# ehsan5890/optical-rl-gym-qot-aware

Hardware: AMD Instinct MI355X
Metric: env steps/sec (whole node) + blocking-prob parity, NSFNET RMSA 320 slots (higher is better)
Workload: dtype u64 bitmap + f64 statistics

## Files before the change

### optical-rl-gym-qot-aware_amd/csrc/orlg_api_step.hip

```cpp
#include "orlg_rmsa_host.h"
#include "orlg_step_call.h"
#include "orlg_qdesc.h"

typedef orlg_rmsa_kernel_t rmsa_kernel_t;

static OrlgGroupOverrides group_overrides() {
    const char *wpb = getenv("ORLG_GROUP_WPB"), *chunks = getenv("ORLG_GROUP_CHUNKS");
    return {getenv("ORLG_NO_DEFER") != nullptr, getenv("ORLG_NO_CHUNKS") != nullptr, getenv("ORLG_NO_LEAN") != nullptr,
            wpb ? atoi(wpb) : 0, chunks ? atoi(chunks) : 0};
}

static bool usage_launch(const OrlgParams &p) {
    return (p.out_mask & ORLG_OUT_ASSIGN_BIT) != 0 && (p.assign == ORLG_ASSIGN_MOST_USED || p.policy == ORLG_POLICY_BEST_WINDOW);
}

static int launch_rmsa_group(orlg_env *e, const OrlgParams &p, const OrlgGroupOverrides &ov) {
    OrlgGroupChoice c = orlg_group_choose(e->group, {p.B, p.n_steps, p.stats_level, p.policy, p.out_mask, p.br_width}, ov, e->num_cu);
    const OrlgGroupLayout &l = e->group[c.kind];
    const bool df = c.kind == ORLG_GROUP_DEFER;
    const bool trace = p.tr_arrival != nullptr;
    const bool traffic = !trace && p.rates != nullptr;
    const bool cause = (p.out_mask & ORLG_OUT_CAUSE_BIT) != 0;
    const bool assign = (p.out_mask & ORLG_OUT_ASSIGN_BIT) != 0;
    const bool cut = assign && p.assign == ORLG_ASSIGN_MIN_CUT;
    const bool usage = usage_launch(p);
    const OrlgGroupKey key = {p.stats_level, c.kind == ORLG_GROUP_HBMQ, df, traffic, trace, cause, assign, cut, usage};
    rmsa_kernel_t k = orlg_pick(e->W, key);
    if (!k) return fail(ORLG_ERR_INVALID, "no kernel for W=%d", e->W);
    if (usage) {
        c.wpb = orlg_group_usage_wpb(l, c.wpb, e->W);
        if (c.wpb < 1)
            return fail(ORLG_ERR_INVALID, "step_kernel \"group\": one wave's four environments (%d B) and their slot-usage prefix sums (%d B) do not "
                                          "fit the LDS next to the tables (%d B); use step_kernel \"wave\" or \"auto\" for this policy",
                        l.wave_bytes, 4 * ORLG_USAGE_BYTES(e->W), l.shared_bytes);
        c.lds_bytes = orlg_group_lds(l.shared_bytes, c.wpb, l.wave_bytes + 4 * ORLG_USAGE_BYTES(e->W));
    }
    if (df && !e->llog)
        if (int rc = orlg_handle_alloc(e, &e->llog, (size_t)p.B * p.E * ORLG_LLOG_CAP)) return rc;
    if (int rc = orlg_kernel_lds(reinterpret_cast<const void *>(k), usage ? c.lds_bytes : orlg_group_lds(l.shared_bytes, l.wpb_max, l.wave_bytes))) return rc;
    int *resident = usage ? &e->group_usage_resident[c.wpb] : &e->group_resident[c.kind][c.wpb];
    if (int rc = orlg_handle_resident(e, reinterpret_cast<const void *>(k), ORLG_WAVE * c.wpb, c.lds_bytes, resident)) return rc;
    const OrlgGroupTickets t = orlg_group_tickets(c, p.B, p.n_steps, *resident, ov);
    if (t.n_chunks > 1) {
        if (!e->progress)
            if (int rc = orlg_handle_alloc(e, &e->progress, (size_t)p.B / 4 + 1)) return rc;
        HIP_TRY(hipMemsetAsync(e->progress, 0, (size_t)t.n_quads * sizeof(uint32_t), e->stream));
    }
    OrlgParams q = p;
    q.llog = df ? e->llog : nullptr;
    q.g_lstat = l.lstat; q.g_lint = l.lint; q.g_qtime = l.qtime; q.g_qdesc = l.qdesc; q.g_wave_bytes = l.wave_bytes;
// ... 403 lines not shown
```

### optical-rl-gym-qot-aware_amd/csrc/orlg_group_body.h

```cpp
    static_assert(!DEFER || (STATS >= 2 && !HBMQ), "the deferred link statistics belong to long launches with full statistics");
    static_assert(!(TRACE && TRAFFIC), "a trace handle has no arrival rates");
    static_assert(!LEAN || DEFER, "the lean body belongs to the long launches");
    static_assert(!CAUSE || (!HBMQ && !DEFER), "the blocking cause belongs to the plain kind");
    static_assert(!ASSIGN || (!HBMQ && !DEFER), "the assignment rules belong to the plain kind");
    static_assert(!CUT || ASSIGN, "the fewest-cuts window is an assignment rule");
    static_assert(!USAGE || (ASSIGN && !CUT), "most-used windows and the best-window route are assignment rules of their own");
    extern __shared__ __align__(16) unsigned char smem[];
    stage_tables(smem, p);
    const int lane = threadIdx.x & 63;
    const int wib = uni((int)(threadIdx.x >> 6));
    const int g = lane >> 4, gl = lane & 15;
    const Tab tb = make_tab(smem, p);
    uint32_t *mt_lds = reinterpret_cast<uint32_t *>(smem + p.l_shared_bytes);
    int *mt_lock = reinterpret_cast<int *>(smem + p.l_shared_bytes + p.g_mt);
    if (threadIdx.x == 0) *mt_lock = 0;
    __syncthreads();
    unsigned char *wbase = smem + p.l_shared_bytes + p.g_mt + 16 + (size_t)wib * p.g_wave_bytes;
    u64 *occ = reinterpret_cast<u64 *>(wbase + p.g_occ) + g * p.NW;
    double *qtime = nullptr;
    uint32_t *qdesc = nullptr;
    if constexpr (!HBMQ) {
        qtime = reinterpret_cast<double *>(wbase + p.g_qtime) + g * p.Q;
        qdesc = reinterpret_cast<uint32_t *>(wbase + p.g_qdesc) + g * p.Q;
    }
    double *lst = DEFER ? nullptr : reinterpret_cast<double *>(wbase + p.g_lstat) + g * 4 * p.E;
    int32_t *lint = reinterpret_cast<int32_t *>(wbase + p.g_lint) + g * p.lint_stride;
    u64 *lsum = DEFER ? reinterpret_cast<u64 *>(wbase + p.g_lstat) + g * p.E : nullptr;

    const int E = p.E, S = p.S, K = p.K, N = p.N, NBR = p.NBR, Q = p.Q, NW = p.NW;
    constexpr bool NET = STATS >= 1;
    constexpr bool FULL = STATS >= 2;
    const double INF = __longlong_as_double((long long)ORLG_INF_BITS);
    const bool out_comp = !LEAN && (p.out_mask & ((1 << ORLG_OUT_COMPACT) | (1 << ORLG_OUT_COMPACT_DIFF))) != 0;
    SEC_DECL_G

    const int n_quads = (p.B + ORLG_GE - 1) / ORLG_GE;
    const int n_chunks = p.n_chunks > 1 ? p.n_chunks : 1;
    const int n_tix = n_quads * n_chunks;
    const int n_waves = (int)(gridDim.x * (blockDim.x >> 6));
// ... 24 lines not shown
        __builtin_amdgcn_fence(__ATOMIC_ACQUIRE, "agent");
        asm volatile("s_waitcnt vmcnt(0)" ::: "memory");
    }
    const int env_raw = quad * ORLG_GE + g;
    const bool act = env_raw < p.B;
    const int env = act ? env_raw : p.B - 1;

    const int env0 = quad * ORLG_GE;
    const int nact = p.B - env0 < ORLG_GE ? p.B - env0 : ORLG_GE;
    quad_copy(wbase + p.g_occ, p.occ + (size_t)env0 * NW, nact * NW * 8, lane);
    if (FULL && !DEFER) quad_copy(wbase + p.g_lstat, p.lstat + (size_t)env0 * 4 * E, nact * 4 * E * 8, lane);
    int32_t *ghist = p.hist + (size_t)env * 4 * NBR;
    [[maybe_unused]] char *hist_q = reinterpret_cast<char *>(p.hist + (size_t)env0 * 4 * NBR);
    [[maybe_unused]] const uint32_t hist_row = (uint32_t)((env - env0) * 4 * NBR) * 4u;
    [[maybe_unused]] auto hist_at = [&](int which, int i) -> int32_t * {
        return reinterpret_cast<int32_t *>(hist_q + (hist_row + (uint32_t)(which * NBR + i) * 4u));
    };
    if (NET) quad_copy(wbase + p.g_lint, p.lint + (size_t)env0 * p.lint_stride, nact * p.lint_stride * 4, lane);
    if (nact < ORLG_GE) {
        wave_sync();
        if (!act) {
            const int gs_ = nact - 1;
            for (int i = gl; i < NW; i += ORLG_GL) occ[i] = (reinterpret_cast<u64 *>(wbase + p.g_occ) + gs_ * NW)[i];
            if (FULL && !DEFER) for (int i = gl; i < 4 * E; i += ORLG_GL) lst[i] = (reinterpret_cast<double *>(wbase + p.g_lstat) + gs_ * 4 * E)[i];
            if (NET) for (int i = gl; i < p.lint_stride; i += ORLG_GL) lint[i] = (reinterpret_cast<int32_t *>(wbase + p.g_lint) + gs_ * p.lint_stride)[i];
        }
    }
    uint4 *llog = DEFER ? p.llog + (size_t)env * E * ORLG_LLOG_CAP : nullptr;
    if (DEFER) lst = p.lstat + (size_t)env * 4 * E;
    bool need_replay = false;
    const OrlgEnvScalars *gs = p.scal + env;
    double current_time = gs->current_time, req_arrival = gs->req_arrival, req_holding = gs->req_holding;
    double g_thr = gs->g_throughput, g_comp = gs->g_compactness, g_lu = gs->g_last_update;
    long long cnt = gs->c[gl & 7];
    long long sum_bitrate_running = gs->sum_bitrate_running, episodes_done = gs->episodes_done;
    int sum_sh = gs->sum_slots_hops, n_running = gs->n_running;
    int req_src = gs->req_src, req_dst = gs->req_dst, req_br = gs->req_br, req_sid = gs->req_sid;
    int mt_idx = gs->mt_idx, new_service = gs->new_service, q_overflow = gs->q_overflow;
    int ring_pos = gs->ring_pos, ring_cnt = gs->ring_cnt;
    int sum_span = gs->sum_span, sum_gaps = gs->sum_gaps;
    int eproc = (int)gs->c[2];
    wave_sync();
    [[maybe_unused]] OrlgGraphEntry lg = {0.0, 0u, 0u, 0u};
    [[maybe_unused]] int lg_cnt = 0;
    double comp_cur = 1.0;
    if (NET && !LEAN) comp_cur = network_compactness(sum_span, sum_sh, sum_gaps, E);
    if (DEFER)
        group_link_stats<W, true, false, true, 2>(lane, occ, nullptr, lint, tb, S, E, nullptr, E, 0.0, sum_span, sum_gaps, comp_cur,
                                                  0, 0.0, g_thr, g_comp, g_lu, nullptr, nullptr, lsum);
    int q_head = gs->q_head, q_n = n_running < Q ? n_running : Q;
    const int q_head0 = q_head;
    int q_pops = 0;
    if constexpr (HBMQ) {
        qtime = p.qtime + (size_t)env * Q;
        qdesc = p.qdesc + (size_t)env * Q;
    } else {
        const double *gqt = p.qtime + (size_t)env * Q;
        const uint32_t *gqd = p.qdesc + (size_t)env * Q;
        for (int j = gl; j < q_n; j += 2 * ORLG_GL) {
            int pos = q_head + j;
            pos -= pos >= Q ? Q : 0;
            int pos2 = pos + ORLG_GL;
            pos2 -= pos2 >= Q ? Q : 0;
            const bool two = j + ORLG_GL < q_n;
            const double t0 = gqt[pos];
            const uint32_t d0 = gqd[pos];
            double t1 = 0.0;
            uint32_t d1 = 0u;
            if (two) { t1 = gqt[pos2]; d1 = gqd[pos2]; }
            qtime[pos] = t0; qdesc[pos] = d0;
            if (two) { qtime[pos2] = t1; qdesc[pos2] = d1; }
        }
    }
    wave_sync();
    double next_rel = q_n > 0 ? qtime[q_head] : INF;
// ... 188 lines not shown
        const double prev_compact = comp_cur;
        bool accepted = false;
        const bool in_range = act && a_path >= 0 && a_path < K && a_slot >= 0 && a_slot < S;
        const int gid = base + (in_range ? a_path : 0);
        const OrlgPathRec *rec = tb.recs + gid;
        int hops = ff_hops, n = ff_n;
        if (LEAN || policy != ORLG_POLICY_EXT) {
            accepted = in_range;
        } else {
            hops = rec->hops;
            n = tb.nslots[req_br * ORLG_NSLOT_STRIDE + rec->se];
            const bool on = in_range && gl < W;
            const u64 x = path_word<W>(occ, tb.recs, gid, gl < W ? gl : 0, on);
            const u64 m = on ? window_mask(a_slot, n, gl) : 0ull;
            const uint32_t bad = row_ballot((x & m) != m, lane);
            accepted = in_range && a_slot + n <= S && bad == 0u;
        }
        const int br_val = tb.bit_rates[req_br];
        [[maybe_unused]] int cause = 0;
        if constexpr (CAUSE) {
            const bool refused = act && !accepted;
            if (ballot(refused) != 0ull) {
                const int level = group_fit_level<W>(lane, occ, tb, base, K, S, req_br, refused);
                cause = refused ? ORLG_CAUSE_CAPACITY + level : ORLG_CAUSE_ACCEPTED;
            }
            if (act) cause_cnt += gl == cause ? 1 : 0;
        }
        if (!NET) group_apply_window<W>(lane, occ, rec->link, accepted ? hops : 0, a_slot, n, false);
        if constexpr (DEFER) vm_drain();
        if (accepted) {
            sum_sh += n * hops;
            n_running += 1;
            sum_bitrate_running += br_val;
            cnt += (cidx == 1 || cidx == 3) ? 1 : ((cidx == 5 || cidx == 7) ? br_val : 0);
            if constexpr (DEFER) {
                if (gl == 0) { atomicAdd(hist_at(1, req_br), 1); atomicAdd(hist_at(3, req_br), 1); }
            } else {
                if (gl == 0) { atomicAdd(ghist + NBR + req_br, 1); atomicAdd(ghist + 3 * NBR + req_br, 1); }
            }
        }
        SEC(4);
        if (NET)
            group_link_stats<W, FULL, !LEAN, DEFER, DEFER ? 1 : 0, true>(lane, occ, lst, lint, tb, S, E, rec->link, accepted ? hops : 0,
                                                                           current_time, sum_span, sum_gaps, comp_cur, sum_sh,
                                                                           (double)sum_bitrate_running, g_thr, g_comp, g_lu, llog,
                                                                           &need_replay, lsum, a_slot, n);
        if constexpr (LEAN) {
            const bool logs = accepted && hops > 0;
            OrlgGraphEntry ne;
            orlg_glog_pack(ne, current_time, sum_bitrate_running, sum_span, sum_sh, sum_gaps);
            if (logs && gl == lg_cnt) lg = ne;
            lg_cnt += logs ? 1 : 0;
            if (ballot(lg_cnt >= ORLG_GLOG_CAP) != 0ull) {
                SEC(15);
                group_graph_replay(lane, lg, lg_cnt, p.scal + env, E);
                vm_drain();
            }
        }
        SEC(5);
        {
            const double rel = req_arrival + req_holding;
            bool ins = accepted && (act || !HBMQ);
            if (ins && q_n >= Q) { q_overflow = 1; ins = false; }
            bool down = false;
            if constexpr (!HBMQ) {
                if (ins && q_n > 0) {
                    int pm = q_head + (q_n >> 1);
                    pm -= pm >= Q ? Q : 0;
                    down = rel < qtime[pm];
                }
            }
            bool found = !ins || q_n == 0;
            int m = q_n;
            int left = q_n;
            int j = down ? gl : q_n - 1 - gl;
            int hd = down ? q_head - 1 : q_head + 1;
            hd = hd < 0 ? Q - 1 : (hd == Q ? 0 : hd);
            while (ballot(!found) != 0ull) {
                const bool scan = !found;
                const bool valid = scan && gl < left;
                int pos = q_head + j;
                pos -= pos >= Q ? Q : 0;
                double tq = 0.0;
// ... 90 lines not shown
                                                  arrival_lambda, holding_lambda)
                    : refill_requests<false>(mt_lds, p.ring_iat + (size_t)env_s * ORLG_RING, p.ring_ht + (size_t)env_s * ORLG_RING,
                                             p.ring_req + (size_t)env_s * ORLG_RING, tb.src_cum, tb.dst_cum, tb.br_cum, &idx_s, N,
                                             NBR, arrival_lambda, holding_lambda, env_s);
                m0 = l_mt[lane]; m1 = l_mt[lane + 64];
                if (lane < 156 - 128) m2 = l_mt[lane + 128];
                __builtin_amdgcn_fence(__ATOMIC_RELEASE, "workgroup");
                if (lane == 0) atomicExch(mt_lock, 0);
                uint4 *o_mt = reinterpret_cast<uint4 *>(p.mt + (size_t)env_s * ORLG_MT_N);
                o_mt[lane] = m0; o_mt[lane + 64] = m1;
                if (lane < 156 - 128) o_mt[lane + 128] = m2;
                ring_visible();
                if constexpr (DEFER) vm_drain();
                if ((lane & 48) == src_lane) { ring_cnt = got; ring_pos = 0; mt_idx = idx_s; dry = false; }
            }
            SEC(7);
            double r_iat = pf_iat, r_ht = pf_ht;
            uint32_t rq = pf_rq;
            if (!pf_ok) {
                const size_t ro = (size_t)env * ORLG_RING + ring_pos;
                r_iat = p.ring_iat[ro]; r_ht = p.ring_ht[ro]; rq = p.ring_req[ro];
                if constexpr (DEFER) vm_drain();
            }
            if (act) {
                const double at = TRACE ? r_iat : current_time + r_iat;
                ring_pos += 1; ring_cnt -= 1;
                current_time = at;
                req_src = (int)(rq & 0xffu); req_dst = (int)((rq >> 8) & 0xffu); req_br = (int)(rq >> 16);
                req_base = tb.pair_base[req_src * N + req_dst];
                req_sid = eproc;
                new_service = 1;
                eproc += 1;
                req_arrival = at; req_holding = r_ht;
                const int bv = tb.bit_rates[req_br];
                cnt += (cidx == 0 || cidx == 2) ? 1 : ((cidx == 4 || cidx == 6) ? bv : 0);
                if constexpr (DEFER) {
                    if (gl == 0) { atomicAdd(hist_at(0, req_br), 1); atomicAdd(hist_at(2, req_br), 1); }
                } else {
                    if (gl == 0) { atomicAdd(ghist + req_br, 1); atomicAdd(ghist + 2 * NBR + req_br, 1); }
                }
            }

            bool released = false;
            for (;;) {
                SEC(9);
                const bool rel_now = act && next_rel <= current_time;
                if (ballot(rel_now) == 0ull) break;
                SEC(10);
                if constexpr (DEFER) {
                    const uint32_t d_a = rel_now ? next_desc : 0u;
                    const uint4 rec_a = *reinterpret_cast<const uint4 *>(tb.recs + (int)(d_a & 0x3fff));
                    double b_rel = INF;
                    uint32_t b_desc = 0u;
                    if (rel_now && q_n >= 2) {
                        const int qb = q_head + 1 == Q ? 0 : q_head + 1;
                        b_rel = qtime[qb]; b_desc = qdesc[qb];
                    }
                    const bool b_due = b_rel <= current_time;
                    const int bri_a = (int)(d_a >> 24);
                    int r_link, r_hop, r_hops, r_s, r_n, pops, br_out, sh_out;
                    if (ballot(b_due) == 0ull) {
                        r_hops = rel_now ? (int)(rec_a.x & 0xffu) : 0;
                        r_n = tb.nslots[bri_a * ORLG_NSLOT_STRIDE + (int)((rec_a.x >> 8) & 0xffu)];
                        br_out = tb.bit_rates[bri_a];
                        r_link = group_rec_byte(rec_a, (gl + 2) & 15);
                        r_hop = gl;
                        r_s = (int)((d_a >> 14) & 0x3ff);
                        pops = 1;
                        sh_out = r_n * r_hops;
                    } else {
                        const bool up = gl >= 8;
                        const bool mine = up ? b_due : rel_now;
// ... 3 lines not shown
                        const OrlgPathRec *rec2 = tb.recs + (int)(d & 0x3fff);
                        const int hops2 = mine ? (int)rec2->hops : 0;
                        const int n2 = tb.nslots[bri2 * ORLG_NSLOT_STRIDE + rec2->se];
                        const int br2 = mine ? tb.bit_rates[bri2] : 0;
                        const int link2 = (int)rec2->link[hop];
                        const u64 lbits = half_row_or_u64(hop < hops2 ? 1ull << (link2 & 63) : 0ull);
                        const u64 obits = ((u64)(uint32_t)row_swap8_i32((int)(uint32_t)(lbits >> 32)) << 32) | (uint32_t)row_swap8_i32((int)(uint32_t)lbits);
                        const int hops_o = row_swap8_i32(hops2), n_o = row_swap8_i32(n2), br_o = row_swap8_i32(br2);
                        const bool pair = b_due && hops2 <= 8 && hops_o <= 8 && (lbits & obits) == 0ull;
                        const bool a_up = up && !pair;
                        const int hops_a = up ? hops_o : hops2, n_a = up ? n_o : n2, br_a = up ? br_o : br2;
                        const int hops_b = up ? hops2 : hops_o, n_b = up ? n2 : n_o, br_b = up ? br2 : br_o;
                        r_link = a_up ? group_rec_byte(rec_a, (gl + 2) & 15) : link2;
                        r_hop = pair ? hop : gl;
                        r_hops = a_up ? hops_a : hops2;
                        r_s = a_up ? (int)((d_a >> 14) & 0x3ff) : s0;
                        r_n = a_up ? n_a : n2;
                        pops = pair ? 2 : 1;
                        br_out = br_a + (pair ? br_b : 0);
                        sh_out = n_a * hops_a + (pair ? n_b * hops_b : 0);
                    }
                    if (rel_now) {
                        q_head += pops;
                        q_head -= q_head >= Q ? Q : 0;
                        q_pops += pops;
                        q_n -= pops;
                        n_running -= pops;
                        sum_bitrate_running -= br_out;
                        sum_sh -= sh_out;
                        released = true;
                        next_rel = q_n > 0 ? qtime[q_head] : INF;
                        next_desc = q_n > 0 ? qdesc[q_head] : 0u;
                    }
                    group_release_links<W>(lane, occ, lsum, lint, S, r_link, r_hop, r_hops, r_s, r_n, current_time, sum_span, sum_gaps,
                                           llog, need_replay);
                    SEC(11);
                } else {
                    const uint32_t d = rel_now ? next_desc : 0u;
                    const int gid2 = (int)(d & 0x3fff), s0 = (int)((d >> 14) & 0x3ff), bri2 = (int)(d >> 24);
                    const OrlgPathRec *rec2 = tb.recs + gid2;
                    const int hops2 = rec2->hops;
                    const int n2 = tb.nslots[bri2 * ORLG_NSLOT_STRIDE + rec2->se];
                    if (rel_now) {
                        if (HBMQ && gl == 0) { qtime[q_head] = INF; qdesc[q_head] = 0u; }
                        q_head = q_head + 1 == Q ? 0 : q_head + 1;
                        q_pops += 1;
                        q_n -= 1;
                        n_running -= 1;
                        sum_bitrate_running -= tb.bit_rates[bri2];
                        sum_sh -= n2 * hops2;
                        released = true;
                    }
                    group_apply_window<W>(lane, occ, rec2->link, rel_now ? hops2 : 0, s0, n2, true);
                    if (rel_now) {
                        next_rel = q_n > 0 ? qtime[q_head] : INF;
                        next_desc = q_n > 0 ? qdesc[q_head] : 0u;
                    }
                    SEC(11);
                    if (NET)
                        group_link_stats<W, FULL, false, DEFER>(lane, occ, lst, lint, tb, S, E, rec2->link, rel_now ? hops2 : 0,
                                                                current_time, sum_span, sum_gaps, comp_cur, sum_sh, 0.0, g_thr, g_comp,
                                                                g_lu, llog, &need_replay);
                }
                if (DEFER && ballot(need_replay) != 0ull) {
                    SEC(14);
                    group_link_replay(lane, lst, lint, tb, S, E, llog);
                    vm_drain();
                    need_replay = false;
                    SEC(11);
                }
            }
            if (NET && out_comp && released) comp_cur = network_compactness(sum_span, sum_sh, sum_gaps, E);
        }

        if (DEFER && ballot(need_replay) != 0ull) {
            SEC(14);
            group_link_replay(lane, lst, lint, tb, S, E, llog);
            vm_drain();
            need_replay = false;
        }
        SEC(12);
        {
            const bool done = act && eproc == p.episode_length;
            if (!LEAN && act && gl == 0 && (p.out_mask & (1 << ORLG_OUT_DONE)))
                ORLG_GPTR(uint8_t, tb.outs[ORLG_OUT_DONE])[(size_t)(t0 + t) * p.B + env] = done ? 1 : 0;
            if (ballot(done && p.auto_reset)) {
                if (done && p.auto_reset) {
                    if constexpr (DEFER) {
                        for (int i = gl; i < NBR; i += ORLG_GL) { atomicExch(hist_at(2, i), 0); atomicExch(hist_at(3, i), 0); }
                    } else {
                        for (int i = gl; i < NBR; i += ORLG_GL) { atomicExch(ghist + 2 * NBR + i, 0); atomicExch(ghist + 3 * NBR + i, 0); }
                    }
                    eproc = 1;
                    episodes_done += 1;
                    const int bv = tb.bit_rates[req_br];
                    if (cidx == 2) cnt = 1;
                    if (cidx == 3 || cidx == 7) cnt = 0;
                    if (cidx == 6) cnt = bv;
                }
                wave_sync();
                if constexpr (DEFER) {
                    if (done && p.auto_reset && gl == 0) atomicExch(hist_at(2, req_br), 1);
                } else {
                    if (done && p.auto_reset && gl == 0) atomicExch(ghist + 2 * NBR + req_br, 1);
                }
                wave_sync();
            }
        }
    }

    SEC(14);
    if (DEFER) group_link_replay(lane, lst, lint, tb, S, E, llog);
    if constexpr (LEAN) {
        SEC(15);
        if (ballot(lg_cnt > 0) != 0ull) group_graph_replay(lane, lg, lg_cnt, p.scal + env, E);
    }
    SEC(13);
    wave_sync();
    {
        const int env0 = quad * ORLG_GE;
        const int nact = p.B - env0 < ORLG_GE ? p.B - env0 : ORLG_GE;
        quad_copy(p.occ + (size_t)env0 * NW, wbase + p.g_occ, nact * NW * 8, lane);
        if (FULL && !DEFER) quad_copy(p.lstat + (size_t)env0 * 4 * E, wbase + p.g_lstat, nact * 4 * E * 8, lane);
        if (NET) quad_copy(p.lint + (size_t)env0 * p.lint_stride, wbase + p.g_lint, nact * p.lint_stride * 4, lane);
    }
    if constexpr (CAUSE) {
        if (act && gl < ORLG_NUM_CAUSES && cause_cnt && p.o_cause_counts) atomicAdd(p.o_cause_counts + (size_t)env * ORLG_NUM_CAUSES + gl, cause_cnt);
    }
    if (act) {
        int q_headc = q_head;
        if constexpr (!HBMQ) {
            double *gqt = p.qtime + (size_t)env * Q;
            uint32_t *gqd = p.qdesc + (size_t)env * Q;
            q_headc = q_head0 + (int)((uint32_t)q_pops % (uint32_t)Q);
            q_headc -= q_headc >= Q ? Q : 0;
            int span = q_pops + q_n;
            span = span > Q ? Q : span;
            for (int j = gl; j < span; j += ORLG_GL) {
                int pos = q_head0 + j;
                pos -= pos >= Q ? Q : 0;
                int i = pos - q_headc;
                i += i < 0 ? Q : 0;
                int src = q_head + i;
                src -= src >= Q ? Q : 0;
                double tq = INF;
                uint32_t dq = 0u;
                if (i < q_n) { tq = qtime[src]; dq = qdesc[src]; }
                gqt[pos] = tq; gqd[pos] = dq;
            }
        }
        OrlgEnvScalars *go = p.scal + env;
        if (gl < 8) go->c[gl] = cnt;
        if (gl == 8) {
            go->current_time = current_time;
            go->req_arrival = req_arrival; go->req_holding = req_holding;
            if (!LEAN) { go->g_throughput = g_thr; go->g_compactness = g_comp; go->g_last_update = g_lu; }
            go->sum_bitrate_running = sum_bitrate_running;
            go->episodes_done = episodes_done;
            go->sum_slots_hops = sum_sh; go->n_running = n_running;
            go->req_src = req_src; go->req_dst = req_dst; go->req_br = req_br; go->req_sid = req_sid;
            go->mt_idx = mt_idx; go->new_service = new_service; go->q_overflow = q_overflow;
            go->ring_pos = ring_pos; go->ring_cnt = ring_cnt;
            go->sum_span = sum_span; go->sum_gaps = sum_gaps; go->q_head = q_headc;
            if (q_overflow) *p.err_flag = 1;
        }
    }
    wave_sync();
    if (n_chunks > 1) {
        asm volatile("s_waitcnt vmcnt(0)" ::: "memory");
        __builtin_amdgcn_fence(__ATOMIC_RELEASE, "agent");
        asm volatile("s_waitcnt vmcnt(0)" ::: "memory");
        if (lane == 0) __hip_atomic_store(p.progress + quad, (uint32_t)(chunk + 1), __ATOMIC_RELAXED, __HIP_MEMORY_SCOPE_AGENT);
    }
    SEC(0);
    }
    SEC_FLUSH;
```

### optical-rl-gym-qot-aware_amd/csrc/orlg_group_kernels.hip

```cpp
#pragma once
#include "orlg_link_stats.h"
#include "orlg_requests.h"
#include "orlg_sections.h"
#include "orlg_block_cause.h"
#include "orlg_assign.h"
#include "orlg_cut.h"
#include "orlg_usage.h"
#include "orlg_graph_log.h"

#define ORLG_GL 16
#define ORLG_GE 4

DEV int row_add_i32(int v) { v += dpp_xor1(v); v += dpp_xor2(v); v += dpp_half_mirror(v); v += dpp_row_mirror(v); return v; }
DEV int row_swap8_i32(int v) { return __builtin_amdgcn_update_dpp(0, v, 0x128, 0xf, 0xf, false); }
DEV u64 half_row_or_u64(u64 v) {
    uint32_t lo = (uint32_t)v, hi = (uint32_t)(v >> 32);
    lo |= (uint32_t)dpp_xor1((int)lo); hi |= (uint32_t)dpp_xor1((int)hi);
    lo |= (uint32_t)dpp_xor2((int)lo); hi |= (uint32_t)dpp_xor2((int)hi);
    lo |= (uint32_t)dpp_half_mirror((int)lo); hi |= (uint32_t)dpp_half_mirror((int)hi);
    return ((u64)hi << 32) | lo;
}
DEV int row_min_i32(int v) {
    int o = dpp_xor1(v); v = o < v ? o : v;
    o = dpp_xor2(v); v = o < v ? o : v;
    o = dpp_half_mirror(v); v = o < v ? o : v;
    o = dpp_row_mirror(v); return o < v ? o : v;
}
DEV uint32_t row_ballot(bool p, int lane) { return (uint32_t)(ballot(p) >> (lane & 48)) & 0xffffu; }

#define ORLG_SEG_REDUCE(name, OP)                                                                   \
    template <int W>                                                                                \
    DEV uint32_t name(uint32_t v) {                                                                 \
        static_assert(W >= 1 && W <= 8 && W != 7, "words per link");                                \
        if (W == 1) return v;                                                                       \
        uint32_t o = (uint32_t)lane_ahead_i32<1>((int)v);                                           \
        const uint32_t s = OP(v, o);                                              \
        if (W == 2) return s;                                                                       \
        o = (uint32_t)lane_ahead_i32<2>((int)(W == 3 ? v : s));                                     \
        const uint32_t t = OP(s, o);                                      \
        if (W <= 4) return t;                                                                       \
        o = (uint32_t)lane_ahead_i32<4>((int)(W == 5 ? v : (W == 6 ? s : t)));                      \
        return OP(t, o);                                                      \
    }
#define ORLG_OP_ADD(a, b) ((a) + (b))
#define ORLG_OP_MAX(a, b) ((a) > (b) ? (a) : (b))
ORLG_SEG_REDUCE(seg_add, ORLG_OP_ADD)
// ... 40 lines not shown
    return (u64)((uint32_t)freec | ((uint32_t)F << 10) | ((uint32_t)U << 20)) |
           ((u64)((uint32_t)(lmin & 0x3ff) | ((uint32_t)lmax << 10) | ((uint32_t)ml << 20) | ((uint32_t)ff << 30) | ((uint32_t)lf << 31)) << 32);
}

template <int W>
DEV bool group_path_candidate(const int lane, const u64 *lsum, const Tab &tb, int gid, int gid0, int w, bool on, int br, uint4 &rec, int &n) {
    constexpr int NH = (ORLG_MAX_HOPS + W - 1) / W;
    const uint32_t *sum_hi = reinterpret_cast<const uint32_t *>(lsum) + 1;
    const OrlgPathRec *pr = tb.recs + (on ? gid : gid0);
    uint4 r = *reinterpret_cast<const uint4 *>(pr);
    int lk[NH];
#pragma unroll
    for (int j = 0; j < NH; ++j) {
        int h = w + j * W;
        if ((j + 1) * W > ORLG_MAX_HOPS) h = h < ORLG_MAX_HOPS - 1 ? h : ORLG_MAX_HOPS - 1;
        lk[j] = (int)pr->link[h];
    }
    n = tb.nslots[br * ORLG_NSLOT_STRIDE + (int)((r.x >> 8) & 0xffu)];
    uint32_t ml = 0x3ffu;
#pragma unroll
    for (int j = 0; j < NH; ++j) {
        const uint32_t m = (sum_hi[2 * lk[j]] >> 20) & 0x3ffu;
        ml = m < ml ? m : ml;
    }
    const uint32_t bad = row_ballot(on && (int)ml < n, lane);
    const uint32_t mine = ((1u << W) - 1u) << ((lane & 15) - w);
    const bool ok = on && (bad & mine) == 0u;
    r.x = ok ? r.x : 0u;
    n = ok ? n : 1;
    rec = r;
    return ok;
}

template <int W, bool LINKF, bool GRAPH, bool DEFER = false, int SUM = 0, bool APPLY = false>
DEV void group_link_stats(const int lane, u64 *occ, double *lst, int32_t *lint, const Tab &tb, int S, int E, const uint8_t *links,
                          int nlinks, double now, int &sum_span, int &sum_gaps, double &comp_cur, int sum_sh, double cur_thr,
                          double &g_thr, double &g_comp, double &g_lu, uint4 *llog = nullptr, bool *need_replay = nullptr,
                          u64 *lsum = nullptr, int win_s = 0, int win_n = 0) {
    static_assert(W <= 8, "at least two links per row");
    static_assert(!APPLY || SUM != 2, "the summary rebuild changes no occupancy");
    static_assert(SUM == 0 || (LINKF && DEFER && (SUM == 1 || !GRAPH)), "summaries belong to the deferred instantiation");
    constexpr int NS = ORLG_GL / W;
    const int gl = lane & 15;
    const int sl = gl / W, w = gl - sl * W;
    double ynow = 0.0;
    if ((LINKF || GRAPH) && nlinks > 0 && now > 0) ynow = recip_refine(now);
    for (int h0 = 0;; h0 += NS) {
        if (ballot(h0 < nlinks) == 0ull) break;
        const int h = h0 + sl;
        const bool on = sl < NS && h < nlinks;
        int link = 0;
        uint32_t packed = 0u, ilo = 0u, hi = 0u, ml = 0u;
        if (on) link = SUM == 2 ? h : (int)links[h];
        u64 x = 0ull;
        if (on) x = occ[__mul24(link, W) + w];
        if (APPLY && on) {
            const u64 m = window_mask(win_s, win_n, w);
            x &= ~m;
            if (m) occ[__mul24(link, W) + w] = x;
        }
        const u64 prev = lane_prev_u64(x);
        int e = 0;
        if (LINKF) {
            const int lead = x == ~0ull ? 64 : ctz64(~x);
            const int nlead_raw = lane_next_i32(lead);
            const int nlead = w < W - 1 ? nlead_raw : 0;
            e = nlead;
// ... 27 lines not shown
                    const uint32_t len = (uint32_t)free_run_length((~x) >> b, 64 - b + e);
                    ml = len > ml ? len : ml;
                }
            }
        }
        packed = seg_add<W>(packed);
        const int lmin = 0x7fff - (int)seg_max<W>(ilo), lmax = (int)seg_max<W>(hi);
        if (LINKF) ml = seg_max<W>(ml);
        const int freec = (int)(packed & 0x3ff), F = (int)((packed >> 10) & 0x3ff), U = (int)(packed >> 20);
        const bool link_lane = on && w == 0;
        if (SUM != 0 && link_lane) lsum[link] = lsum_pack(freec, F, U, lmin, lmax, (int)ml, first_free, last_free);
        if (SUM == 2) { wave_sync(); continue; }
        int dspan = 0, dgaps = 0;
        if (link_lane) {
            int nspan = U > 1 ? lmax - lmin : 0, ngaps = U > 1 ? U - 1 : 0;
            int old = lint[link];
            int cnt = 0;
            if (LINKF && DEFER) {
                cnt = (int)((uint32_t)old >> 26);
                const int max_empty = (F > 1 && !(F == 2 && first_free && last_free)) ? (int)ml : 0;
                if (cnt < ORLG_LLOG_CAP - 1) {
                    llog[__mul24(link, ORLG_LLOG_CAP) + cnt] =
                        make_uint4((uint32_t)freec | ((uint32_t)max_empty << 10) | ((uint32_t)(lmax - lmin) << 20), (uint32_t)U,
                                   (uint32_t)__double2loint(now), (uint32_t)__double2hiint(now));
                    cnt += 1;
                }
                if (cnt >= ORLG_LLOG_FLUSH) *need_replay = true;
                old &= 0x03ffffff;
            }
            lint[link] = nspan | (ngaps << 16) | (cnt << 26);
            dspan = nspan - (old & 0xffff);
            dgaps = ngaps - (old >> 16);
        }
        sum_span += row_add_i32(dspan);
        sum_gaps += row_add_i32(dgaps);
        if (LINKF && !DEFER && link_lane && now > 0) {
            double *l_util = lst, *l_ef = lst + E, *l_c = lst + 2 * E, *l_lu = lst + 3 * E;
            const double last_update = l_lu[link];
            const double last0 = l_util[link], last1 = l_ef[link], last2 = l_c[link];
            const double cur0 = tb.div_s[S - freec];
            double cur1 = 0.0, cur2 = 0.0;
            if (freec > 0) {
                int max_empty = (F > 1 && !(F == 2 && first_free && last_free)) ? (int)ml : 0;
                cur1 = 1.0 - ORLG_FDIV((double)max_empty, (double)freec);
                cur2 = U > 1 ? ORLG_FDIV((double)(lmax - lmin), (double)(S - freec)) * tb.inv_k[U] : 1.0;
            }
            const double time_diff = now - last_update;
            l_util[link] = div_by((last0 * last_update) + (cur0 * time_diff), now, ynow);
            l_ef[link] = div_by((last1 * last_update) + (cur1 * time_diff), now, ynow);
            l_c[link] = div_by((last2 * last_update) + (cur2 * time_diff), now, ynow);
        }
        if (LINKF && !DEFER && link_lane) lst[3 * E + link] = now;
        wave_sync();
    }
    if (GRAPH && SUM != 2 && nlinks > 0) {
        comp_cur = network_compactness(sum_span, sum_sh, sum_gaps, E);
        if (now > 0) {
            const double time_diff = now - g_lu;
            g_thr = div_by((g_thr * g_lu) + (cur_thr * time_diff), now, ynow);
            g_comp = div_by((g_comp * g_lu) + (comp_cur * time_diff), now, ynow);
        }
        g_lu = now;
    }
}

template <int W>
DEV void group_release_links(const int lane, u64 *occ, u64 *lsum, int32_t *lint, int S, const int link, int hop, int hops, int s,
                             int n, double now, int &sum_span, int &sum_gaps, uint4 *llog, bool &need_replay) {
    static_assert(ORLG_MAX_HOPS <= ORLG_GL, "one lane per hop");
    int dspan = 0, dgaps = 0;
    if (hop < hops) {
        u64 *lw = occ + __mul24(link, W);
        const int e = s + n;
        const int ia = s > 0 ? (s - 1) >> 6 : 0, ib = e < S ? e >> 6 : 0, ws = s >> 6, we = (e - 1) >> 6;
        const u64 xa = lw[ia], xb = lw[ib], xs = lw[ws], xe = lw[we];
        const u64 sm = lsum[link];
        const u64 hm = ~0ull << (s & 63), lm = ~0ull >> (63 - ((e - 1) & 63));
        if (ws == we) {
            lw[ws] = xs | (hm & lm);
        } else {
            lw[ws] = xs | hm;
            for (int j = ws + 1; j < we; ++j) lw[j] = ~0ull;
            lw[we] = xe | lm;
        }
        int p = -1, q = 64 * W;
        if (s > 0) {
            const u64 y = ~xa & (~0ull >> (63 - ((s - 1) & 63)));
            if (y) p = 64 * ia + 63 - clz64(y);
            else
                for (int j = ia - 1; j >= 0; --j) {
                    const u64 v = ~lw[j];
                    if (v) { p = 64 * j + 63 - clz64(v); break; }
                }
        }
        if (e < S) {
            const u64 y = ~xb & (~0ull << (e & 63));
            if (y) q = 64 * ib + ctz64(y);
            else
                for (int j = ib + 1; j < W; ++j) {
// ... 5 lines not shown
        }
        const int L = s - 1 - p, R = q - e;
        const uint32_t lo32 = (uint32_t)sm, hi32 = (uint32_t)(sm >> 32);
        const int freec = (int)(lo32 & 0x3ff) + n;
        const int F = (int)((lo32 >> 10) & 0x3ff) + 1 - (L > 0) - (R > 0);
        const int U = (int)((lo32 >> 20) & 0x3ff) + (s > 0 && L == 0) + (e < S && R == 0) - 1;
        int lmin = (int)(hi32 & 0x3ff);
        int lmax = (int)((hi32 >> 10) & 0x3ff);
        int ml = (int)((hi32 >> 20) & 0x3ff);
        const bool ff = ((hi32 >> 30) & 1u) || s == 0, lf = (hi32 >> 31) || e == S;
        ml = L + n + R > ml ? L + n + R : ml;
        if (U == 0) { lmin = 0x7fff; lmax = 0; }
        else {
            if (lmin == s) lmin = e + R;
            if (lmax == e) lmax = s - L;
        }
        lsum[link] = lsum_pack(freec, F, U, lmin, lmax, ml, ff, lf);
        const int nspan = U > 1 ? lmax - lmin : 0, ngaps = U > 1 ? U - 1 : 0;
        int old = lint[link];
        int cnt = (int)((uint32_t)old >> 26);
        const int max_empty = (F > 1 && !(F == 2 && ff && lf)) ? ml : 0;
        if (cnt < ORLG_LLOG_CAP - 1) {
            llog[__mul24(link, ORLG_LLOG_CAP) + cnt] =
                make_uint4((uint32_t)freec | ((uint32_t)max_empty << 10) | ((uint32_t)(lmax - lmin) << 20), (uint32_t)U,
                           (uint32_t)__double2loint(now), (uint32_t)__double2hiint(now));
            cnt += 1;
        }
        if (cnt >= ORLG_LLOG_FLUSH) need_replay = true;
        old &= 0x03ffffff;
        lint[link] = nspan | (ngaps << 16) | (cnt << 26);
        dspan = nspan - (old & 0xffff);
        dgaps = ngaps - (old >> 16);
    }
    sum_span += row_add_i32(dspan);
    sum_gaps += row_add_i32(dgaps);
    wave_sync();
}

DEV void group_link_replay(const int lane, double *lst, int32_t *lint, const Tab &tb, int S, int E, const uint4 *llog) {
    link_replay<ORLG_GL>(lane, lst, lint, tb, S, E, llog);
}

static_assert(255 * 64 * ORLG_MAX_W <= ORLG_GLOG_MAX_ES, "a link is a byte, a link's bitmap ORLG_MAX_W words: the log's E S fields");
DEV void group_graph_replay(const int lane, const OrlgGraphEntry &lg, int &cnt, OrlgEnvScalars *gs, int E) {
    const int gl = lane & 15;
    __builtin_amdgcn_fence(__ATOMIC_RELEASE, "workgroup");
    __builtin_amdgcn_fence(__ATOMIC_ACQUIRE, "workgroup");
    const bool head = gl == 0 && cnt > 0;
    double x_thr = 0.0, x_comp = 0.0, g_lu = 0.0;
    if (head) { x_thr = gs->g_throughput; x_comp = gs->g_compactness; g_lu = gs->g_last_update; }
    const double before = ORLG_DPP_F64(lane_prev_i32, lg.now);
    const double lu = gl == 0 ? g_lu : before;
    const OrlgGraphTerm t = orlg_glog_eval(lg, lu, E);
    const bool upd = gl < cnt && t.now > 0;
    const int c0 = __builtin_amdgcn_readlane(cnt, 0), c1 = __builtin_amdgcn_readlane(cnt, 16);
    const int c2 = __builtin_amdgcn_readlane(cnt, 32), c3 = __builtin_amdgcn_readlane(cnt, 48);
    const int m01 = c0 > c1 ? c0 : c1, m23 = c2 > c3 ? c2 : c3;
    const int nmax = m01 > m23 ? m01 : m23;
    double o_thr = 0.0, o_comp = 0.0;
    for (int k = 0; k < nmax; ++k) {
        const double n_thr = orlg_glog_chain(x_thr, lu, t.c_thr, t.now, t.ynow);
        const double n_comp = orlg_glog_chain(x_comp, lu, t.c_comp, t.now, t.ynow);
        o_thr = upd ? n_thr : x_thr;
        o_comp = upd ? n_comp : x_comp;
        x_thr = ORLG_DPP_F64(lane_prev_i32, o_thr);
        x_comp = ORLG_DPP_F64(lane_prev_i32, o_comp);
    }
    if (gl == nmax - 1 && cnt > 0) { gs->g_throughput = o_thr; gs->g_compactness = o_comp; }
// ... 106 lines not shown
```

### optical-rl-gym-qot-aware_amd/csrc/orlg_group_plan.h

```cpp
#pragma once
#include <cmath>
#include <cstddef>

#include "../../include/orlg.h"
#include "orlg_device.h"
#include "orlg_lds.h"

enum OrlgGroupKind { ORLG_GROUP_PLAIN, ORLG_GROUP_HBMQ, ORLG_GROUP_DEFER };
struct OrlgGroupLayout { int occ, lstat, lint, qtime, qdesc, wave_bytes, wpb_max, shared_bytes; };
enum { ORLG_GROUP_MT_BYTES = (ORLG_MT_N * 4 + 15) & ~15 };
static inline size_t orlg_group_lds(size_t shared_bytes, int wpb, int wave_bytes) { return shared_bytes + ORLG_GROUP_MT_BYTES + 16 + (size_t)wpb * wave_bytes; }
static inline OrlgGroupLayout orlg_group_layout(OrlgGroupKind kind, int NW, int E, int Q, int lint_stride, int stats_level, int shared_bytes) {
    auto up16 = [](int v) { return (v + 15) & ~15; };
    OrlgGroupLayout l = {};
    int go = up16(4 * NW * 8);
    l.lstat = go; if (kind != ORLG_GROUP_DEFER && stats_level >= ORLG_STATS_FULL) go = up16(go + 4 * 4 * E * 8);
    l.lint = go; go = up16(go + 4 * lint_stride * 4);
    l.qtime = go; go = up16(go + 4 * Q * 8);
    l.qdesc = go; go = up16(go + 4 * Q * 4);
    if (kind == ORLG_GROUP_DEFER) { l.lstat = go; go = up16(go + 4 * E * 8); }
    l.wave_bytes = kind == ORLG_GROUP_HBMQ ? l.qtime : go;
    l.shared_bytes = shared_bytes;
    for (int cand = ORLG_GROUP_WAVES; cand >= 1 && !l.wpb_max; cand--)
        if (orlg_group_lds(shared_bytes, cand, l.wave_bytes) <= ORLG_LDS_BYTES) l.wpb_max = cand;
    return l;
}

static inline int orlg_group_usage_wpb(const OrlgGroupLayout &l, int wpb, int W) {
    while (wpb >= 1 && orlg_group_lds(l.shared_bytes, wpb, l.wave_bytes + 4 * ORLG_USAGE_BYTES(W)) > ORLG_LDS_BYTES) --wpb;
    return wpb;
}

struct OrlgGroupLaunch { int B, n_steps, stats_level, policy, out_mask, br_width; };
struct OrlgGroupOverrides { bool no_defer, no_chunks, no_lean; int wpb, chunks; };
struct OrlgGroupChoice { OrlgGroupKind kind; int wpb; size_t lds_bytes; bool lean; uint32_t ticket_stride; bool long_rounds; };
struct OrlgGroupTickets { int n_quads, nblocks, n_chunks, chunk_steps; uint32_t ticket_advance; };

static inline bool orlg_defer_link_stats(int stats_level, int n_steps, int out_mask, const OrlgGroupOverrides &ov) {
    return stats_level >= 2 && n_steps >= 16 && !ov.no_defer &&
           !(out_mask & ((1 << ORLG_OUT_AVG_LINK_COMPACT) | (1 << ORLG_OUT_AVG_LINK_UTIL) | ORLG_OUT_PLAIN_BITS));
}

static inline OrlgGroupChoice orlg_group_choose(const OrlgGroupLayout *layouts, const OrlgGroupLaunch &a, const OrlgGroupOverrides &ov, int num_cu) {
    OrlgGroupChoice c = {};
    const bool hq = a.n_steps <= ORLG_DIRECT_STEPS && layouts[ORLG_GROUP_HBMQ].wpb_max > layouts[ORLG_GROUP_PLAIN].wpb_max &&
                    !(a.out_mask & ORLG_OUT_PLAIN_BITS);
    const bool df = !hq && orlg_defer_link_stats(a.stats_level, a.n_steps, a.out_mask, ov) && layouts[ORLG_GROUP_DEFER].wpb_max >= 1;
    c.kind = hq ? ORLG_GROUP_HBMQ : df ? ORLG_GROUP_DEFER : ORLG_GROUP_PLAIN;
    const int wpb_max = layouts[c.kind].wpb_max, n_quads = (a.B + 3) / 4;
    c.wpb = wpb_max;
    c.long_rounds = a.n_steps >= 256 && !hq && n_quads >= wpb_max * num_cu && !ov.no_chunks;
    if (!c.long_rounds) {
        double best = 1e300;
        for (int w = wpb_max; w >= 1; --w) {
            const double rounds = (double)n_quads / ((double)num_cu * w);
            const double cost = ((rounds < 3.0 || a.n_steps <= 16) ? std::ceil(rounds) : rounds + 0.5) * (w + 1.5);
            if (cost < best - 1e-9) { best = cost; c.wpb = w; }
        }
    }
    if (ov.wpb >= 1 && ov.wpb <= wpb_max) c.wpb = ov.wpb;
    c.lds_bytes = orlg_group_lds(layouts[c.kind].shared_bytes, c.wpb, layouts[c.kind].wave_bytes);
    c.lean = df && (a.policy == ORLG_POLICY_SP || a.policy == ORLG_POLICY_SAP) && a.out_mask == 0 && a.br_width == 0 && !ov.no_lean;
    c.ticket_stride = a.n_steps <= 16 ? 1u : 0u;
    return c;
}

static inline OrlgGroupTickets orlg_group_tickets(const OrlgGroupChoice &c, int B, int n_steps, int resident, const OrlgGroupOverrides &ov) {
    OrlgGroupTickets t = {};
    t.n_quads = (B + 3) / 4;
    t.nblocks = (t.n_quads + c.wpb - 1) / c.wpb;
    if (t.nblocks > resident) t.nblocks = resident;
    const int slots = t.nblocks * c.wpb;
    int k = 1;
    if (c.long_rounds && !c.ticket_stride && t.n_quads > slots) {
        k = (int)std::floor(8.0 * slots / t.n_quads + 0.5);
        k = k < 1 ? 1 : (k > 4 ? 4 : k);
        while (k > 1 && n_steps / k < 128) --k;
    }
    if (ov.chunks >= 1 && ov.chunks <= 64 && !c.ticket_stride && c.kind != ORLG_GROUP_HBMQ) k = ov.chunks < n_steps ? ov.chunks : n_steps;
    t.chunk_steps = (n_steps + k - 1) / k;
    t.n_chunks = (n_steps + t.chunk_steps - 1) / t.chunk_steps;
    if (!c.ticket_stride) t.ticket_advance = (uint32_t)t.n_quads * (uint32_t)t.n_chunks + (t.n_chunks > 1 ? (uint32_t)slots : 0u);
    return t;
}
```

Before: 1.894 billion.

## Batch lean-path histogram counters in lane registers and defer span/gap row sums

In the lean deferred-statistics body, per-bit-rate request and acceptance counts are now kept as packed 16-bit counters in per-lane registers. They are flushed to the global histogram and scalar counters with atomics only periodically, on episode reset, and at kernel end, instead of issuing global atomics on every arrival and acceptance. The per-step cross-lane reductions of span and gap deltas are also dropped in favour of per-lane partial sums, which are reduced only when a graph log entry is packed or at write-back. This cuts per-step atomics and DPP reductions in exchange for more bookkeeping code, a cap of 32 bit rates for the lean path, and a 16-bit counter overflow bound tied to the flush interval.

```diff
diff --git a/optical-rl-gym-qot-aware_amd/csrc/orlg_api_step.hip b/optical-rl-gym-qot-aware_amd/csrc/orlg_api_step.hip
--- a/optical-rl-gym-qot-aware_amd/csrc/orlg_api_step.hip
+++ b/optical-rl-gym-qot-aware_amd/csrc/orlg_api_step.hip
@@ -15,7 +15,7 @@
 }
 
 static int launch_rmsa_group(orlg_env *e, const OrlgParams &p, const OrlgGroupOverrides &ov) {
-    OrlgGroupChoice c = orlg_group_choose(e->group, {p.B, p.n_steps, p.stats_level, p.policy, p.out_mask, p.br_width}, ov, e->num_cu);
+    OrlgGroupChoice c = orlg_group_choose(e->group, {p.B, p.n_steps, p.stats_level, p.policy, p.out_mask, p.br_width, p.NBR}, ov, e->num_cu);
     const OrlgGroupLayout &l = e->group[c.kind];
     const bool df = c.kind == ORLG_GROUP_DEFER;
     const bool trace = p.tr_arrival != nullptr;
diff --git a/optical-rl-gym-qot-aware_amd/csrc/orlg_group_body.h b/optical-rl-gym-qot-aware_amd/csrc/orlg_group_body.h
--- a/optical-rl-gym-qot-aware_amd/csrc/orlg_group_body.h
+++ b/optical-rl-gym-qot-aware_amd/csrc/orlg_group_body.h
@@ -5,6 +5,7 @@
     static_assert(!ASSIGN || (!HBMQ && !DEFER), "the assignment rules belong to the plain kind");
     static_assert(!CUT || ASSIGN, "the fewest-cuts window is an assignment rule");
     static_assert(!USAGE || (ASSIGN && !CUT), "most-used windows and the best-window route are assignment rules of their own");
+    constexpr bool LANE_HIST = LEAN, LANE_SUMS = LEAN;
     extern __shared__ __align__(16) unsigned char smem[];
     stage_tables(smem, p);
     const int lane = threadIdx.x & 63;
@@ -95,15 +96,49 @@
     const OrlgEnvScalars *gs = p.scal + env;
     double current_time = gs->current_time, req_arrival = gs->req_arrival, req_holding = gs->req_holding;
     double g_thr = gs->g_throughput, g_comp = gs->g_compactness, g_lu = gs->g_last_update;
-    long long cnt = gs->c[gl & 7];
+    [[maybe_unused]] long long cnt = gs->c[gl & 7];
     long long sum_bitrate_running = gs->sum_bitrate_running, episodes_done = gs->episodes_done;
     int sum_sh = gs->sum_slots_hops, n_running = gs->n_running;
     int req_src = gs->req_src, req_dst = gs->req_dst, req_br = gs->req_br, req_sid = gs->req_sid;
     int mt_idx = gs->mt_idx, new_service = gs->new_service, q_overflow = gs->q_overflow;
     int ring_pos = gs->ring_pos, ring_cnt = gs->ring_cnt;
     int sum_span = gs->sum_span, sum_gaps = gs->sum_gaps;
+    if (LANE_SUMS && gl != 0) { sum_span = 0; sum_gaps = 0; }
     int eproc = (int)gs->c[2];
     wave_sync();
+    [[maybe_unused]] uint32_t h_req = 0u, h_acc = 0u;
+    [[maybe_unused]] auto lane_one = [&](int br) -> uint32_t { return (br & (ORLG_GL - 1)) == gl ? 1u << (br & ORLG_GL) : 0u; };
+    [[maybe_unused]] uint32_t br_one = lane_one(req_br);
+    [[maybe_unused]] auto cold_row = [&]() -> uint32_t {
+        uint32_t r = (uint32_t)(env - env0);
+        asm volatile("" : "+v"(r));
+        return r;
+    };
+    [[maybe_unused]] auto hist_lean = [&](uint32_t row, int which, int i) -> int32_t * {
+        return reinterpret_cast<int32_t *>(reinterpret_cast<char *>(p.hist + (size_t)env0 * 4 * NBR) + ((row * 4u + (uint32_t)which) * (uint32_t)NBR + (uint32_t)i) * 4u);
+    };
+    [[maybe_unused]] auto books_flush = [&](const bool rows, const bool episode) {
+        const int gh = gl + ORLG_GL;
+        const int rate_lo = gl < NBR ? tb.bit_rates[gl] : 0, rate_hi = gh < NBR ? tb.bit_rates[gh] : 0;
+        const int req_lo = (int)(h_req & 0xffffu), req_hi = (int)(h_req >> 16), acc_lo = (int)(h_acc & 0xffffu), acc_hi = (int)(h_acc >> 16);
+        const long long n_req = row_add_i32(req_lo + req_hi), n_acc = row_add_i32(acc_lo + acc_hi);
+        const long long b_req = row_add_i64((long long)req_lo * rate_lo + (long long)req_hi * rate_hi);
+        const long long b_acc = row_add_i64((long long)acc_lo * rate_lo + (long long)acc_hi * rate_hi);
+        if (rows) {
+            const uint32_t row = cold_row();
+            if (gl < NBR && req_lo) { atomicAdd(hist_lean(row, 0, gl), req_lo); atomicAdd(hist_lean(row, 2, gl), req_lo); }
+            if (gh < NBR && req_hi) { atomicAdd(hist_lean(row, 0, gh), req_hi); atomicAdd(hist_lean(row, 2, gh), req_hi); }
+            if (gl < NBR && acc_lo) { atomicAdd(hist_lean(row, 1, gl), acc_lo); atomicAdd(hist_lean(row, 3, gl), acc_lo); }
+            if (gh < NBR && acc_hi) { atomicAdd(hist_lean(row, 1, gh), acc_hi); atomicAdd(hist_lean(row, 3, gh), acc_hi); }
+            if (gl < 8) {
+                int64_t *c = reinterpret_cast<OrlgEnvScalars *>(reinterpret_cast<char *>(p.scal + env0) + row * (uint32_t)sizeof(OrlgEnvScalars))->c + gl;
+                long long v = *c + ((gl & 4) ? ((gl & 1) ? b_acc : b_req) : ((gl & 1) ? n_acc : n_req));
+                if (episode) v = gl == 2 ? 1 : (gl == 6 ? tb.bit_rates[req_br] : ((gl == 3 || gl == 7) ? 0 : v));
+                *c = v;
+            }
+            h_req = 0u; h_acc = 0u;
+        }
+    };
     [[maybe_unused]] OrlgGraphEntry lg = {0.0, 0u, 0u, 0u};
     [[maybe_unused]] int lg_cnt = 0;
     double comp_cur = 1.0;
@@ -358,23 +393,28 @@
             sum_sh += n * hops;
             n_running += 1;
             sum_bitrate_running += br_val;
-            cnt += (cidx == 1 || cidx == 3) ? 1 : ((cidx == 5 || cidx == 7) ? br_val : 0);
-            if constexpr (DEFER) {
-                if (gl == 0) { atomicAdd(hist_at(1, req_br), 1); atomicAdd(hist_at(3, req_br), 1); }
+            if constexpr (LANE_HIST) {
+                h_acc += br_one;
             } else {
-                if (gl == 0) { atomicAdd(ghist + NBR + req_br, 1); atomicAdd(ghist + 3 * NBR + req_br, 1); }
+                cnt += (cidx == 1 || cidx == 3) ? 1 : ((cidx == 5 || cidx == 7) ? br_val : 0);
+                if constexpr (DEFER) {
+                    if (gl == 0) { atomicAdd(hist_at(1, req_br), 1); atomicAdd(hist_at(3, req_br), 1); }
+                } else {
+                    if (gl == 0) { atomicAdd(ghist + NBR + req_br, 1); atomicAdd(ghist + 3 * NBR + req_br, 1); }
+                }
             }
         }
         SEC(4);
         if (NET)
-            group_link_stats<W, FULL, !LEAN, DEFER, DEFER ? 1 : 0, true>(lane, occ, lst, lint, tb, S, E, rec->link, accepted ? hops : 0,
+            group_link_stats<W, FULL, !LEAN, DEFER, DEFER ? 1 : 0, true, LANE_SUMS>(lane, occ, lst, lint, tb, S, E, rec->link, accepted ? hops : 0,
                                                                            current_time, sum_span, sum_gaps, comp_cur, sum_sh,
                                                                            (double)sum_bitrate_running, g_thr, g_comp, g_lu, llog,
                                                                            &need_replay, lsum, a_slot, n);
         if constexpr (LEAN) {
             const bool logs = accepted && hops > 0;
             OrlgGraphEntry ne;
-            orlg_glog_pack(ne, current_time, sum_bitrate_running, sum_span, sum_sh, sum_gaps);
+            orlg_glog_pack(ne, current_time, sum_bitrate_running, LANE_SUMS ? row_add_i32(sum_span) : sum_span, sum_sh,
+                           LANE_SUMS ? row_add_i32(sum_gaps) : sum_gaps);
             if (logs && gl == lg_cnt) lg = ne;
             lg_cnt += logs ? 1 : 0;
             if (ballot(lg_cnt >= ORLG_GLOG_CAP) != 0ull) {
@@ -531,12 +571,17 @@
                 new_service = 1;
                 eproc += 1;
                 req_arrival = at; req_holding = r_ht;
-                const int bv = tb.bit_rates[req_br];
-                cnt += (cidx == 0 || cidx == 2) ? 1 : ((cidx == 4 || cidx == 6) ? bv : 0);
-                if constexpr (DEFER) {
-                    if (gl == 0) { atomicAdd(hist_at(0, req_br), 1); atomicAdd(hist_at(2, req_br), 1); }
+                if constexpr (LANE_HIST) {
+                    br_one = lane_one(req_br);
+                    h_req += br_one;
                 } else {
-                    if (gl == 0) { atomicAdd(ghist + req_br, 1); atomicAdd(ghist + 2 * NBR + req_br, 1); }
+                    const int bv = tb.bit_rates[req_br];
+                    cnt += (cidx == 0 || cidx == 2) ? 1 : ((cidx == 4 || cidx == 6) ? bv : 0);
+                    if constexpr (DEFER) {
+                        if (gl == 0) { atomicAdd(hist_at(0, req_br), 1); atomicAdd(hist_at(2, req_br), 1); }
+                    } else {
+                        if (gl == 0) { atomicAdd(ghist + req_br, 1); atomicAdd(ghist + 2 * NBR + req_br, 1); }
+                    }
                 }
             }
 
@@ -606,7 +651,7 @@
                         next_rel = q_n > 0 ? qtime[q_head] : INF;
                         next_desc = q_n > 0 ? qdesc[q_head] : 0u;
                     }
-                    group_release_links<W>(lane, occ, lsum, lint, S, r_link, r_hop, r_hops, r_s, r_n, current_time, sum_span, sum_gaps,
+                    group_release_links<W, LANE_SUMS>(lane, occ, lsum, lint, S, r_link, r_hop, r_hops, r_s, r_n, current_time, sum_span, sum_gaps,
                                            llog, need_replay);
                     SEC(11);
                 } else {
@@ -659,26 +704,42 @@
             if (!LEAN && act && gl == 0 && (p.out_mask & (1 << ORLG_OUT_DONE)))
                 ORLG_GPTR(uint8_t, tb.outs[ORLG_OUT_DONE])[(size_t)(t0 + t) * p.B + env] = done ? 1 : 0;
             if (ballot(done && p.auto_reset)) {
+                if constexpr (LANE_HIST) books_flush(done && p.auto_reset, true);
                 if (done && p.auto_reset) {
-                    if constexpr (DEFER) {
+                    if constexpr (LANE_HIST) {
+                        const uint32_t row = cold_row();
+                        for (int i = gl; i < NBR; i += ORLG_GL) { atomicExch(hist_lean(row, 2, i), 0); atomicExch(hist_lean(row, 3, i), 0); }
+                    } else if constexpr (DEFER) {
                         for (int i = gl; i < NBR; i += ORLG_GL) { atomicExch(hist_at(2, i), 0); atomicExch(hist_at(3, i), 0); }
                     } else {
                         for (int i = gl; i < NBR; i += ORLG_GL) { atomicExch(ghist + 2 * NBR + i, 0); atomicExch(ghist + 3 * NBR + i, 0); }
                     }
                     eproc = 1;
                     episodes_done += 1;
-                    const int bv = tb.bit_rates[req_br];
-                    if (cidx == 2) cnt = 1;
-                    if (cidx == 3 || cidx == 7) cnt = 0;
-                    if (cidx == 6) cnt = bv;
+                    if constexpr (!LANE_HIST) {
+                        const int bv = tb.bit_rates[req_br];
+                        if (cidx == 2) cnt = 1;
+                        if (cidx == 3 || cidx == 7) cnt = 0;
+                        if (cidx == 6) cnt = bv;
+                    }
                 }
                 wave_sync();
-                if constexpr (DEFER) {
+                if constexpr (LANE_HIST) {
+                    if (done && p.auto_reset && gl == 0) atomicExch(hist_lean(cold_row(), 2, req_br), 1);
+                } else if constexpr (DEFER) {
                     if (done && p.auto_reset && gl == 0) atomicExch(hist_at(2, req_br), 1);
                 } else {
                     if (done && p.auto_reset && gl == 0) atomicExch(ghist + 2 * NBR + req_br, 1);
                 }
                 wave_sync();
+                if constexpr (LANE_HIST) vm_drain();
+            }
+        }
+        if constexpr (LANE_HIST) {
+            static_assert(ORLG_LEAN_FLUSH_STEPS < 0x10000 && (ORLG_LEAN_FLUSH_STEPS & (ORLG_LEAN_FLUSH_STEPS - 1)) == 0, "16-bit fields");
+            if ((t & (ORLG_LEAN_FLUSH_STEPS - 1)) == ORLG_LEAN_FLUSH_STEPS - 1) {
+                books_flush(act, false);
+                vm_drain();
             }
         }
     }
@@ -689,6 +750,8 @@
         SEC(15);
         if (ballot(lg_cnt > 0) != 0ull) group_graph_replay(lane, lg, lg_cnt, p.scal + env, E);
     }
+    if constexpr (LANE_HIST) books_flush(act, false);
+    [[maybe_unused]] const int span_row = LANE_SUMS ? row_add_i32(sum_span) : sum_span, gaps_row = LANE_SUMS ? row_add_i32(sum_gaps) : sum_gaps;
     SEC(13);
     wave_sync();
     {
@@ -724,7 +787,9 @@
             }
         }
         OrlgEnvScalars *go = p.scal + env;
-        if (gl < 8) go->c[gl] = cnt;
+        if constexpr (!LANE_HIST) {
+            if (gl < 8) go->c[gl] = cnt;
+        }
         if (gl == 8) {
             go->current_time = current_time;
             go->req_arrival = req_arrival; go->req_holding = req_holding;
@@ -735,7 +800,7 @@
             go->req_src = req_src; go->req_dst = req_dst; go->req_br = req_br; go->req_sid = req_sid;
             go->mt_idx = mt_idx; go->new_service = new_service; go->q_overflow = q_overflow;
             go->ring_pos = ring_pos; go->ring_cnt = ring_cnt;
-            go->sum_span = sum_span; go->sum_gaps = sum_gaps; go->q_head = q_headc;
+            go->sum_span = span_row; go->sum_gaps = gaps_row; go->q_head = q_headc;
             if (q_overflow) *p.err_flag = 1;
         }
     }
diff --git a/optical-rl-gym-qot-aware_amd/csrc/orlg_group_kernels.hip b/optical-rl-gym-qot-aware_amd/csrc/orlg_group_kernels.hip
--- a/optical-rl-gym-qot-aware_amd/csrc/orlg_group_kernels.hip
+++ b/optical-rl-gym-qot-aware_amd/csrc/orlg_group_kernels.hip
@@ -10,8 +10,14 @@
 
 #define ORLG_GL 16
 #define ORLG_GE 4
+#define ORLG_LEAN_FLUSH_STEPS 0x8000
 
 DEV int row_add_i32(int v) { v += dpp_xor1(v); v += dpp_xor2(v); v += dpp_half_mirror(v); v += dpp_row_mirror(v); return v; }
+#define ORLG_DPP_I64(fn, x) (long long)(((u64)(uint32_t)fn((int)((u64)(x) >> 32)) << 32) | (uint32_t)fn((int)(uint32_t)(x)))
+DEV long long row_add_i64(long long v) {
+    v += ORLG_DPP_I64(dpp_xor1, v); v += ORLG_DPP_I64(dpp_xor2, v); v += ORLG_DPP_I64(dpp_half_mirror, v); v += ORLG_DPP_I64(dpp_row_mirror, v);
+    return v;
+}
 DEV int row_swap8_i32(int v) { return __builtin_amdgcn_update_dpp(0, v, 0x128, 0xf, 0xf, false); }
 DEV u64 half_row_or_u64(u64 v) {
     uint32_t lo = (uint32_t)v, hi = (uint32_t)(v >> 32);
@@ -118,7 +124,7 @@
     return ok;
 }
 
-template <int W, bool LINKF, bool GRAPH, bool DEFER = false, int SUM = 0, bool APPLY = false>
+template <int W, bool LINKF, bool GRAPH, bool DEFER = false, int SUM = 0, bool APPLY = false, bool PART = false>
 DEV void group_link_stats(const int lane, u64 *occ, double *lst, int32_t *lint, const Tab &tb, int S, int E, const uint8_t *links,
                           int nlinks, double now, int &sum_span, int &sum_gaps, double &comp_cur, int sum_sh, double cur_thr,
                           double &g_thr, double &g_comp, double &g_lu, uint4 *llog = nullptr, bool *need_replay = nullptr,
@@ -212,8 +218,13 @@
             dspan = nspan - (old & 0xffff);
             dgaps = ngaps - (old >> 16);
         }
-        sum_span += row_add_i32(dspan);
-        sum_gaps += row_add_i32(dgaps);
+        if constexpr (PART) {
+            sum_span += dspan;
+            sum_gaps += dgaps;
+        } else {
+            sum_span += row_add_i32(dspan);
+            sum_gaps += row_add_i32(dgaps);
+        }
         if (LINKF && !DEFER && link_lane && now > 0) {
             double *l_util = lst, *l_ef = lst + E, *l_c = lst + 2 * E, *l_lu = lst + 3 * E;
             const double last_update = l_lu[link];
@@ -244,7 +255,7 @@
     }
 }
 
-template <int W>
+template <int W, bool PART = false>
 DEV void group_release_links(const int lane, u64 *occ, u64 *lsum, int32_t *lint, int S, const int link, int hop, int hops, int s,
                              int n, double now, int &sum_span, int &sum_gaps, uint4 *llog, bool &need_replay) {
     static_assert(ORLG_MAX_HOPS <= ORLG_GL, "one lane per hop");
@@ -316,8 +327,13 @@
         dspan = nspan - (old & 0xffff);
         dgaps = ngaps - (old >> 16);
     }
-    sum_span += row_add_i32(dspan);
-    sum_gaps += row_add_i32(dgaps);
+    if constexpr (PART) {
+        sum_span += dspan;
+        sum_gaps += dgaps;
+    } else {
+        sum_span += row_add_i32(dspan);
+        sum_gaps += row_add_i32(dgaps);
+    }
     wave_sync();
 }
 
diff --git a/optical-rl-gym-qot-aware_amd/csrc/orlg_group_plan.h b/optical-rl-gym-qot-aware_amd/csrc/orlg_group_plan.h
--- a/optical-rl-gym-qot-aware_amd/csrc/orlg_group_plan.h
+++ b/optical-rl-gym-qot-aware_amd/csrc/orlg_group_plan.h
@@ -31,7 +31,8 @@
     return wpb;
 }
 
-struct OrlgGroupLaunch { int B, n_steps, stats_level, policy, out_mask, br_width; };
+enum { ORLG_LEAN_MAX_BIT_RATES = 32 };
+struct OrlgGroupLaunch { int B, n_steps, stats_level, policy, out_mask, br_width, n_bit_rates = 0; };
 struct OrlgGroupOverrides { bool no_defer, no_chunks, no_lean; int wpb, chunks; };
 struct OrlgGroupChoice { OrlgGroupKind kind; int wpb; size_t lds_bytes; bool lean; uint32_t ticket_stride; bool long_rounds; };
 struct OrlgGroupTickets { int n_quads, nblocks, n_chunks, chunk_steps; uint32_t ticket_advance; };
@@ -60,7 +61,8 @@
     }
     if (ov.wpb >= 1 && ov.wpb <= wpb_max) c.wpb = ov.wpb;
     c.lds_bytes = orlg_group_lds(layouts[c.kind].shared_bytes, c.wpb, layouts[c.kind].wave_bytes);
-    c.lean = df && (a.policy == ORLG_POLICY_SP || a.policy == ORLG_POLICY_SAP) && a.out_mask == 0 && a.br_width == 0 && !ov.no_lean;
+    c.lean = df && (a.policy == ORLG_POLICY_SP || a.policy == ORLG_POLICY_SAP) && a.out_mask == 0 && a.br_width == 0 && !ov.no_lean &&
+             a.n_bit_rates <= ORLG_LEAN_MAX_BIT_RATES;
     c.ticket_stride = a.n_steps <= 16 ? 1u : 0u;
     return c;
 }
```

After: 1.964 billion (median of 6 runs). +3.7%, better.
